# moskewcz/boda

Measured on AMD Instinct MI355X. Metric: effective TFLOP/s (2*M*N*K / time), whole job, higher is better.
Workload: dtype f32

## Files before the change

### boda_amd/csrc/kernels/sgemm_big_f32.hip

```cpp

#ifndef __HIPCC_RTC__
#include <hip/hip_runtime.h>
#endif

typedef float f32x16 __attribute__((ext_vector_type(16)));
typedef float f32x4 __attribute__((ext_vector_type(4)));
typedef unsigned u32x2 __attribute__((ext_vector_type(2)));
#ifndef GROUP_I
#define GROUP_I 8
#endif
#ifndef BKS
#define BKS 8
#endif
#ifndef PF
#define PF 2
#endif
#ifndef TBI
#define TBI 256
#endif
#ifndef TBJ
#define TBJ 256
#endif
#ifndef WI
#define WI 2
#endif
#ifndef WJ
#define WJ 4
#endif
#ifndef MINW
#define MINW 1
#endif
#ifndef MULPRIO
#define MULPRIO 1
#endif
#ifndef STGPRIO
#define STGPRIO 0
#endif
#ifndef NSTG
#define NSTG 4
#endif

struct gemm_args_t {
  float const *I; float const *J; float *D; float const *bias;
  int Mi, Nj, K;
  int ldI, ldJ, ldD;
  int C, H, W, OH, OW;
  int tiles_i, tiles_j;
  int splitk, kt_per;
  float *ws; long ws_slab;
  unsigned I_bytes, J_bytes;
  unsigned D_bytes;
  int out_ctot, out_coff;
  int const *ktab; int ktab_n;
  long bsI, bsJ, bsD;
};

namespace {
constexpr int kNMW = WI * WJ;
static_assert(kNMW == 8 || kNMW == 4, "eight (or four) multiplying waves");
constexpr int kTI = TBI / (WI * 32), kTJ = TBJ / (WJ * 32);
static_assert(TBI % (WI * 32) == 0 && TBJ % (WJ * 32) == 0 && (kTI == 4 || kTI == 2 || kTI == 1) && (kTJ == 2 || kTJ == 1), "wave tile: 4 | 2 | 1 row blocks x 2 | 1 column blocks");
constexpr int kLDI = TBI + 4, kLDJ = TBJ + 4;
constexpr int kImgI = BKS * kLDI, kImgJ = BKS * kLDJ, kImg2 = kImgI + kImgJ;
constexpr int kNLI = BKS * (TBI / 4) / 256, kNLJ = BKS * (TBJ / 4) / 256;
static_assert((BKS * (TBI / 4)) % 256 == 0 && (BKS * (TBJ / 4)) % 256 == 0, "whole float4 units per staging thread");
constexpr int kKK = BKS / 2;
constexpr int kU = (NSTG == 3) ? 3 * PF : ((PF > NSTG) ? PF : NSTG);
constexpr int kD = NSTG - 1;
static_assert(NSTG == 3 || NSTG == 4, "NSTG: 3 | 4");
constexpr int kOOB = (int)0x80000000;
static_assert(BKS % 4 == 0 && (PF == 2 || PF == 4), "BKS % 4 == 0, PF: 2 | 4");
typedef __amdgpu_buffer_rsrc_t rsrc_t;
__device__ __forceinline__ rsrc_t make_rsrc(float const *p, unsigned bytes) { return __builtin_amdgcn_make_buffer_rsrc((void *)p, 0, (int)bytes, 0x00020000); }
__device__ __forceinline__ f32x4 bload4(rsrc_t r, int voff, int soff) { return __builtin_bit_cast(f32x4, __builtin_amdgcn_raw_buffer_load_b128(r, voff, soff, 0)); }
}

#if (TBI / (WI * 32)) == 4
typedef f32x4 avec_t;
#elif (TBI / (WI * 32)) == 2
typedef float2 avec_t;
#else
typedef float avec_t;
#endif
#if (TBJ / (WJ * 32)) == 2
typedef float2 bvec_t;
#else
typedef float bvec_t;
#endif
namespace {
__device__ __forceinline__ float vget(f32x4 const &v, int i) { return v[i]; }
__device__ __forceinline__ float vget(float2 const &v, int i) { return i ? v.y : v.x; }
__device__ __forceinline__ float vget(float const &v, int) { return v; }
}

extern "C" __global__ __launch_bounds__((kNMW + 4) * 64, MINW) void KNAME(gemm_args_t const p) {
  __shared__ __attribute__((aligned(16))) float sm[NSTG * kImg2];
  int const lane = threadIdx.x & 63;
  int const wave = __builtin_amdgcn_readfirstlane(threadIdx.x >> 6);
  bool const stager = wave >= kNMW;

  int tile_i, tile_j;
  {
    int const bid = blockIdx.x, nb = p.tiles_i * p.tiles_j;
    int const q = nb >> 3, rr = nb & 7, xcd = bid & 7, idx = bid >> 3;
    int const nid = ((xcd < rr) ? xcd * (q + 1) : rr * (q + 1) + (xcd - rr) * q) + idx;
    int const group_sz = GROUP_I * p.tiles_j, gid = nid / group_sz, first_i = gid * GROUP_I;
    int const gsz = min(p.tiles_i - first_i, GROUP_I), in_g = nid - gid * group_sz;
    tile_i = first_i + in_g % gsz; tile_j = in_g / gsz;
  }
  int const i0 = tile_i * TBI, j0 = tile_j * TBJ;
  int const nkt = (p.K + BKS - 1) / BKS;
  int const nkt_pad = (nkt + kU - 1) / kU * kU;

  if (stager) {
#if STGPRIO
    __builtin_amdgcn_s_setprio(STGPRIO);
#endif
    int const tid = threadIdx.x - kNMW * 64;
    rsrc_t const rI = make_rsrc(p.I, p.I_bytes), rJ = make_rsrc(p.J, p.J_bytes);
    int goffI[kNLI], goffJ[kNLJ], loffI[kNLI], loffJ[kNLJ], krowI[kNLI], krowJ[kNLJ];
#pragma unroll
    for (int n = 0; n < kNLI; ++n) {
      int const c = tid + n * 256, kr = c / (TBI / 4), x = 4 * (c % (TBI / 4));
      krowI[n] = kr; loffI[n] = kr * kLDI + x;
      goffI[n] = (i0 + x < p.Mi) ? ((kr * p.ldI + i0 + x) * 4) : kOOB;
    }
#pragma unroll
    for (int n = 0; n < kNLJ; ++n) {
      int const c = tid + n * 256, kr = c / (TBJ / 4), x = 4 * (c % (TBJ / 4));
      krowJ[n] = kr; loffJ[n] = kImgI + kr * kLDJ + x;
      goffJ[n] = (j0 + x < p.Nj) ? ((kr * p.ldJ + j0 + x) * 4) : kOOB;
    }
    auto gloadI = [&](int n, int kt) -> f32x4 { return bload4(rI, (kt * BKS + krowI[n] < p.K) ? goffI[n] : kOOB, min(kt, nkt - 1) * (BKS * 4) * p.ldI); };
    auto gloadJ = [&](int n, int kt) -> f32x4 { return bload4(rJ, (kt * BKS + krowJ[n] < p.K) ? goffJ[n] : kOOB, min(kt, nkt - 1) * (BKS * 4) * p.ldJ); };
    auto lstoreI = [&](int n, int stage, f32x4 const &v) { *reinterpret_cast<f32x4 *>(sm + stage * kImg2 + loffI[n]) = v; };
    auto lstoreJ = [&](int n, int stage, f32x4 const &v) { *reinterpret_cast<f32x4 *>(sm + stage * kImg2 + loffJ[n]) = v; };
    f32x4 ringI[PF][kNLI], ringJ[PF][kNLJ];
#pragma unroll
    for (int u = 0; u < PF; ++u) {
#pragma unroll
      for (int n = 0; n < kNLI; ++n) ringI[u][n] = gloadI(n, u);
#pragma unroll
      for (int n = 0; n < kNLJ; ++n) ringJ[u][n] = gloadJ(n, u);
    }
#pragma unroll
    for (int t = 0; t < kD; ++t) {
#pragma unroll
      for (int n = 0; n < kNLI; ++n) { lstoreI(n, t, ringI[t % PF][n]); ringI[t % PF][n] = gloadI(n, t + PF); }
#pragma unroll
      for (int n = 0; n < kNLJ; ++n) { lstoreJ(n, t, ringJ[t % PF][n]); ringJ[t % PF][n] = gloadJ(n, t + PF); }
    }
    asm volatile("s_waitcnt lgkmcnt(0)\n s_barrier" ::: "memory");
    for (int kb = 0; kb < nkt_pad; kb += kU) {
#pragma unroll
      for (int u = 0; u < kU; ++u) {
#pragma unroll
        for (int n = 0; n < kNLI; ++n) { lstoreI(n, (u + kD) % NSTG, ringI[(u + kD) % PF][n]); ringI[(u + kD) % PF][n] = gloadI(n, kb + u + kD + PF); }
#pragma unroll
        for (int n = 0; n < kNLJ; ++n) { lstoreJ(n, (u + kD) % NSTG, ringJ[(u + kD) % PF][n]); ringJ[(u + kD) % PF][n] = gloadJ(n, kb + u + kD + PF); }
        asm volatile("s_waitcnt lgkmcnt(%0)\n s_barrier" :: "n"(kNLI + kNLJ) : "memory");
      }
    }
    return;
  }

#if MULPRIO
  __builtin_amdgcn_s_setprio(MULPRIO);
#endif
  int const wi = wave / WJ, wj = wave % WJ;
  float const *const a_base = sm + (lane >> 5) * kLDI + wi * (kTI * 32) + kTI * (lane & 31);
  float const *const b_base = sm + kImgI + (lane >> 5) * kLDJ + wj * (kTJ * 32) + kTJ * (lane & 31);
  f32x16 acc[kTI][kTJ];
#pragma unroll
  for (int t = 0; t < kTI; ++t)
#pragma unroll
    for (int u = 0; u < kTJ; ++u)
#pragma unroll
      for (int r = 0; r < 16; ++r) acc[t][u][r] = 0.f;

  asm volatile("s_barrier" ::: "memory");
  avec_t a[2]; bvec_t b[2];
  a[0] = *reinterpret_cast<avec_t const *>(a_base); b[0] = *reinterpret_cast<bvec_t const *>(b_base);
  static_assert(kKK % 2 == 0, "an even number of k pairs per step (the operand double buffer carries over from step to step)");
  for (int kb = 0; kb < nkt_pad; kb += kU) {
#pragma unroll
    for (int s = 0; s < kU; ++s) {
      float const *const A = a_base + (s % NSTG) * kImg2, *const B = b_base + (s % NSTG) * kImg2;
      float const *const An = a_base + ((s + 1) % NSTG) * kImg2, *const Bn = b_base + ((s + 1) % NSTG) * kImg2;
#pragma unroll
      for (int kk = 0; kk < kKK; ++kk) {
        if (kk + 1 < kKK) { a[(kk + 1) & 1] = *reinterpret_cast<avec_t const *>(A + (kk + 1) * 2 * kLDI); b[(kk + 1) & 1] = *reinterpret_cast<bvec_t const *>(B + (kk + 1) * 2 * kLDJ); }
#if NSTG == 4
        else { a[0] = *reinterpret_cast<avec_t const *>(An); b[0] = *reinterpret_cast<bvec_t const *>(Bn); }
#endif
        __builtin_amdgcn_sched_barrier(0);
        avec_t const ca = a[kk & 1]; bvec_t const cb = b[kk & 1];
#pragma unroll
        for (int t = 0; t < kTI; ++t)
#pragma unroll
          for (int u = 0; u < kTJ; ++u) acc[t][u] = __builtin_amdgcn_mfma_f32_32x32x2f32(vget(ca, t), vget(cb, u), acc[t][u], 0, 0, 0);
        __builtin_amdgcn_sched_barrier(0);
      }
#if NSTG == 4
      asm volatile("s_barrier" ::: "memory");
#else
      asm volatile("s_waitcnt lgkmcnt(0)\n s_barrier" ::: "memory");
      a[0] = *reinterpret_cast<avec_t const *>(An); b[0] = *reinterpret_cast<bvec_t const *>(Bn);
#endif
    }
  }

  {
    rsrc_t const rD = make_rsrc(p.D, p.D_bytes);
    int const j = j0 + wj * (kTJ * 32) + kTJ * (lane & 31);
    int const il = i0 + wi * (kTI * 32) + kTI * 4 * (lane >> 5);
#pragma unroll
    for (int t = 0; t < kTI; ++t)
#pragma unroll
      for (int r = 0; r < 16; ++r) {
        int const i = il + kTI * ((r & 3) + 8 * (r >> 2)) + t;
        int const off = ((i < p.Mi) && (j < p.Nj)) ? ((i * p.ldD + j) * 4) : kOOB;
#if (TBJ / (WJ * 32)) == 2
        float2 const v = float2{acc[t][0][r], acc[t][1][r]};
        __builtin_amdgcn_raw_buffer_store_b64(__builtin_bit_cast(u32x2, v), rD, off, 0, 0);
#else
        float const v = acc[t][0][r];
        __builtin_amdgcn_raw_buffer_store_b32(__builtin_bit_cast(unsigned, v), rD, off, 0, 0);
#endif
      }
  }
}
```

### boda_amd/csrc/native_internal.h

```cpp
#pragma once
#include "native_kernels.h"
#include <algorithm>
#include <cstdlib>
#include <sstream>

namespace bodahip {

struct gemm_args_t {
  float const *I; float const *J; float *D; float const *bias;
  int Mi, Nj, K;
  int ldI, ldJ, ldD;
  int C, H, W, OH, OW;
  int tiles_i, tiles_j;
  int splitk, kt_per;
  float *ws; long ws_slab;
  unsigned I_bytes, J_bytes;
  unsigned D_bytes;
  int out_ctot, out_coff;
  void const *ktab; int ktab_n;
  long bsI, bsJ, bsD;
};
struct chain_args_t : gemm_args_t {
  float const *I2; float const *bias2; float *Dmid;
  int M2; unsigned I2_bytes, Dmid_bytes;
};
static_assert(sizeof(gemm_args_t) == 176, "gemm_args_t is declared with this size by every kernel source (and by set_kernel_source's text)");

struct kernel_t { hipModule_t mod = nullptr; hipFunction_t func = nullptr; int occ = 0; };

struct native_kernels_t::impl_t {
  std::map<string, kernel_t> kernels;
  std::map<string, string> tune;
  void *ws = nullptr; size_t ws_bytes = 0;
  std::vector<void *> ws_retired;
  std::map<string, void *> ktabs;
  int call_ws_hold = 0;
  size_t call_ws_bytes = 0;
  size_t ts_off = 0, ts_bytes = 0; string ts_hdr;
  hipModule_t wino_mod = nullptr; hipFunction_t wino_filt = nullptr, wino_in = nullptr, wino_out = nullptr, wino_fused = nullptr, wino_filt_t = nullptr;
};


struct plan_t { tile_cfg_t cfg; vect_string defs; string kname; long split_pels = 0; tile_cfg_t tail_cfg; vect_string tail_defs;    bool ipconv = false, k1 = false, bf16 = false, patch = false, stream = false, quad = false, fc = false, big = false, cbig = false, rdec = false, patch16 = false, nhwc = false, nhwc_patch = false, nhwc_multi = false, nhwc_rows = false, ksl = false, bconv_in = false, bconv_filts = false; int rows = 0, cg = 0; };

struct bconv_args_t {
  float const *a; float const *b; float *d;
  float *ws; long ws_slab;
  int B, C, H, W, OC, OH, OW;
  int tiles_i, tiles_j, ksl, kt_per;
  unsigned a_bytes, b_bytes, d_bytes;
};
// ... 50 lines not shown
```

### boda_amd/csrc/native_kernels.cc

```cpp
#include "native_internal.h"

namespace bodahip {

#include "kernels_embed.inc"

native_kernels_t::native_kernels_t(native_host_t *host_) : impl(new impl_t), host(host_) {
  if (char const *e = getenv("BODAHIP_SGEMM_TILE")) impl->tune["sgemm_tile"] = e;
  if (char const *e = getenv("BODAHIP_CONV_TILE")) impl->tune["conv_tile"] = e;
  if (char const *e = getenv("BODAHIP_K1_STREAM")) impl->tune["k1_stream"] = e;
  if (char const *e = getenv("BODAHIP_CONV_ALGO")) impl->tune["conv_algo"] = e;
  if (char const *e = getenv("BODAHIP_EXACT")) impl->tune["exact"] = e;
}
native_kernels_t::~native_kernels_t() {
  if (impl->ts_bytes && impl->ws) {
    char const *e = getenv("BODAHIP_CBIG_TSTAMP"); string fn = e ? string(e) : string(); if (fn.size() > 5 && fn.substr(fn.size() - 5) == ":late") fn.resize(fn.size() - 5);
    std::vector<unsigned long long> h(impl->ts_bytes / 8);
    if (!fn.empty() && hipDeviceSynchronize() == hipSuccess && hipMemcpy(h.data(), (char *)impl->ws + impl->ts_off, impl->ts_bytes, hipMemcpyDeviceToHost) == hipSuccess) {
      if (FILE *f = fopen(fn.c_str(), "a")) { fprintf(f, "%s\n", impl->ts_hdr.c_str());
        for (size_t w = 0; w < h.size() / 16; ++w) { for (int e2 = 0; e2 < 16; ++e2) fprintf(f, "%llu ", h[w * 16 + e2]); fprintf(f, "\n"); } fclose(f); }
    }
  }
  for (auto &kv : impl->kernels) { if (kv.second.mod) (void)hipModuleUnload(kv.second.mod); }
  if (impl->wino_mod) (void)hipModuleUnload(impl->wino_mod);
  if (impl->ws) (void)hipFree(impl->ws);
// ... 10 lines not shown
void native_kernels_t::check_compile_time(rtc_func_info_t const &fi) {
  string const &fn = fi.op.get_func_name();
  if (fn == "hip_sgemm" || fn == "cublas_sgemm" || fn == "hip_sgemm_bf16") return;
  if (fn == "hip_conv" || fn == "cudnn_conv" || fn == "hip_conv_bf16" || fn == "hip_conv_winograd" || fn == "hip_conv_nhwc" || fn == "hip_conv_nhwc_grp" || fn == "hip_conv_nhwc_multi" || fn == "hip_conv_nhwc_set") { (void)fi.op.get_u32("conv_has_relu"); return; }
  if (fn == "hip_conv_k1_chain") { (void)fi.op.get_u32("conv_has_relu"); (void)fi.op.get_u32("conv_has_relu2"); return; }
  if (fn == "hip_conv_filts_kmajor") return;
  if (fn == "hip_bconv_in" || fn == "hip_bconv_filts" || fn == "hip_bconv_biases") {
    for (char const *an : {"in", "filts", "out_grad_loss", "stride", "in_pad"}) (void)fi.op.get_dims(an);
    return;
  }
  rt_err("unknown/unhandled native hip function: " + fn);
}
void native_kernels_t::set_tune(string const &key, string const &val) {
  if (key != "sgemm_tile" && key != "conv_tile" && key != "k1_stream" && key != "conv_algo" && key != "exact") rt_err("set_tune: unknown key '" + key + "'");
  if (key == "exact" && !val.empty() && val != "0" && val != "1") rt_err("set_tune: exact must be 0 | 1");
  if (key == "conv_algo" && !val.empty() && val != "direct" && val != "winograd" && val != "winograd_all") rt_err("set_tune: conv_algo must be direct | winograd | winograd_all");
  if (val.empty()) impl->tune.erase(key); else { impl->tune[key] = val; }
}


void launch(native_host_t *host, kernel_t &k, gemm_args_t &a, tile_cfg_t const &c) {
  void *params[] = {&a};
  uint32_t const grid = (uint32_t)a.tiles_i * (uint32_t)a.tiles_j * (uint32_t)std::max(1, a.splitk);
  hip_err_chk(host->nh_launch(k.func, grid, 1, (uint32_t)c.threads(), params), "hipModuleLaunchKernel(native)");
}


std::vector<char> compile_plan(plan_t const &p, string const &arch, string *log) {
  vect_string opts = p.defs; opts.push_back("-DKNAME=" + p.kname);
  return hiprtc_compile(p.bconv_in ? k_src_bconv_in_f32 : p.bconv_filts ? k_src_bconv_filts_f32 : p.nhwc_rows ? k_src_conv_nhwc_rows_bf16 : p.nhwc_multi ? k_src_conv_nhwc_multi_bf16 : p.nhwc_patch ? k_src_conv_nhwc_patch_bf16 : p.nhwc ? k_src_conv_nhwc_bf16 : p.patch16 ? k_src_conv_patch_bf16 : (p.cbig ? k_src_conv_big_f32 : p.big ? k_src_sgemm_big_f32 : p.fc ? k_src_fc_f32 : p.stream ? (p.quad ? k_src_k1_quad_f32 : k_src_k1_stream_f32) : (p.bf16 ? k_src_gemm_conv_bf16 : k_src_gemm_conv_f32)), p.kname, arch, opts, log, true);
}

void ensure_ws(native_kernels_t::impl_t *impl, native_host_t *host, size_t need) {
  if (impl->ws_bytes >= need) return;
  if (host->nh_capturing()) rt_err("graph capture: kernel workspace not allocated yet -- run the call list once before capturing it");
  if (impl->ws) {
    hip_err_chk(hipStreamSynchronize(host->nh_stream()), "hipStreamSynchronize");
    if (host->nh_live_graphs() > 0) impl->ws_retired.push_back(impl->ws); else hip_err_chk(hipFree(impl->ws), "hipFree");
    impl->ws = nullptr; impl->ws_bytes = 0;
  }
  hip_err_chk(hipMalloc(&impl->ws, need), "hipMalloc(kernel scratch)"); impl->ws_bytes = need;
}
static void setup_splitk(native_kernels_t::impl_t *impl, native_host_t *host, gemm_args_t &ga, tile_cfg_t const &cfg, size_t out_elems) {
  ga.splitk = cfg.SPLITK; ga.kt_per = 0; ga.ws = nullptr; ga.ws_slab = 0;
  if (cfg.SPLITK <= 1) { ga.splitk = 1; return; }
  int const nkt = (ga.K + cfg.BK - 1) / cfg.BK;
  ga.kt_per = (nkt + cfg.SPLITK - 1) / cfg.SPLITK;
// ... 113 lines not shown
  void *d = nullptr;
  hip_err_chk(hipMalloc(&d, h.size() * sizeof(int)), "hipMalloc(rtab)");
  hip_err_chk(hipMemcpyAsync(d, h.data(), h.size() * sizeof(int), hipMemcpyHostToDevice, host->nh_stream()), "hipMemcpyAsync(rtab)");
  hip_err_chk(hipStreamSynchronize(host->nh_stream()), "hipStreamSynchronize");
  impl->ktabs.emplace(key, d);
  return ktab_t{d, (int)n};
}

string tune_of(native_kernels_t::impl_t *impl, char const *key) { auto t = impl->tune.find(key); return (t == impl->tune.end()) ? string() : t->second; }

static void sgemm_parts(native_kernels_t *nk, native_kernels_t::impl_t *impl, native_host_t *host, float const *a, float const *b, float *c, uint32_t M, uint32_t N, uint32_t K, std::vector<sgemm_part_t> const &parts) {
  if ((uint64_t)K * M * 4 > 0x80000000ull || (uint64_t)K * N * 4 > 0x80000000ull || (uint64_t)M * N * 4 >= 0x7ffffff0ull) unsup_err("hip_sgemm: operands / c of 2 GiB or more are not supported (32-bit buffer offsets)");
  uint32_t grid = 0; bool first = true;
  for (sgemm_part_t const &q : parts) {
    plan_t const p = plan_sgemm(q.rows, q.cols, K, host->nh_num_cus(), q.tile, false);
    kernel_t &k = get_kernel(impl, host, p);
    gemm_args_t ga; memset(&ga, 0, sizeof(ga));
    ga.I = a + q.m0; ga.J = b + q.n0; ga.D = c + (size_t)q.m0 * N + q.n0; ga.bias = nullptr;
    ga.Mi = (int)q.rows; ga.Nj = (int)q.cols; ga.K = (int)K; ga.ldI = (int)M; ga.ldJ = (int)N; ga.ldD = (int)N;
    ga.I_bytes = (unsigned)(((uint64_t)K * M - q.m0) * 4); ga.J_bytes = (unsigned)(((uint64_t)K * N - q.n0) * 4); ga.D_bytes = (unsigned)((((uint64_t)q.rows - 1) * N + q.cols) * 4);
    ga.tiles_i = (int)((q.rows + p.cfg.BI - 1) / p.cfg.BI); ga.tiles_j = (int)((q.cols + p.cfg.BJ - 1) / p.cfg.BJ); ga.splitk = 1;
    launch(host, k, ga, p.cfg);
    grid += (uint32_t)ga.tiles_i * ga.tiles_j;
    if (first) { nk->last_launch.kernel = p.kname; nk->last_launch.cfg = p.cfg; nk->last_launch.block = p.cfg.threads(); first = false; }
  }
  nk->last_launch.grid = grid; nk->last_launch.flops = 2.0 * M * N * K; nk->last_launch.algo_bytes = 4.0 * ((double)K * M + (double)K * N + (double)M * N);
}

void native_kernels_t::sgemm(float const *a, float const *b, float *c, uint32_t M, uint32_t N, uint32_t K, bool bf16, bool half) {
  if (!M || !N) return;
  size_t const esz = half ? 2 : 4;
  if (half && bf16) unsup_err("hip_sgemm_bf16: half-typed tensors are not supported (bf16 OPERANDS are made from float tensors)");
  if (!K) { hip_err_chk(hipMemsetAsync(c, 0, (size_t)M * N * esz, host->nh_stream()), "hipMemsetAsync"); return; }
  if (M > 0x7fffffffu || N > 0x7fffffffu || K > 0x7fffffffu) unsup_err("hip_sgemm: dims exceed int32");
  string tile_for;
  if (char const *e = getenv("BODAHIP_SGEMM_TILE_FOR")) {
    string const key = std::to_string(M) + "="; string const v = e; size_t const at = (";" + v).find(";" + key);
    if (M == N && N == K && at != string::npos) { size_t const b = at + key.size(), en = v.find(';', b); tile_for = v.substr(b, en == string::npos ? string::npos : en - b); }
  }
  if (!bf16 && !half && tune_of(impl, "sgemm_tile").empty() && tile_for.empty() && M % 4 == 0 && N % 4 == 0) {
    std::vector<sgemm_part_t> parts;
    if (!parse_parts_env(M, N, K, parts)) parts = plan_sgemm_parts(M, N, K, host->nh_num_cus());
    if (!parts.empty()) { sgemm_parts(this, impl, host, a, b, c, M, N, K, parts); return; }
  }
  if (!bf16 && !half && tune_of(impl, "sgemm_tile").empty() && tile_for.empty()) tile_for = sgemm_wide_tile(M, N, K, host->nh_num_cus());
  if (!bf16 && !half && tune_of(impl, "sgemm_tile").empty() && tile_for.empty()) {
    sgemm_split_t const sp = plan_sgemm_split(M, N, K, host->nh_num_cus());
    if (sp.m_main) {
      if ((uint64_t)K * M * 4 > 0x80000000ull || (uint64_t)K * N * 4 > 0x80000000ull || (uint64_t)M * N * 4 >= 0x7ffffff0ull) unsup_err("hip_sgemm: operands / c of 2 GiB or more are not supported (32-bit buffer offsets)");
      uint32_t grid = 0;
      for (int part = 0; part < 2; ++part) {
        uint32_t const m0 = part ? sp.m_main : 0, rows = part ? M - sp.m_main : sp.m_main;
        plan_t const p = plan_sgemm(rows, N, K, host->nh_num_cus(), part ? sp.tail_tile : string(kBigTile), false);
        kernel_t &k = get_kernel(impl, host, p);
        gemm_args_t ga; memset(&ga, 0, sizeof(ga));
        ga.I = a + m0; ga.J = b; ga.D = c + (size_t)m0 * N; ga.bias = nullptr;
        ga.Mi = (int)rows; ga.Nj = (int)N; ga.K = (int)K; ga.ldI = (int)M; ga.ldJ = (int)N; ga.ldD = (int)N;
        ga.I_bytes = (unsigned)(((uint64_t)K * M - m0) * 4); ga.J_bytes = (unsigned)((uint64_t)K * N * 4); ga.D_bytes = (unsigned)((uint64_t)rows * N * 4);
        ga.tiles_i = (int)((rows + p.cfg.BI - 1) / p.cfg.BI); ga.tiles_j = (int)((N + p.cfg.BJ - 1) / p.cfg.BJ); ga.splitk = 1;
        launch(host, k, ga, p.cfg);
        grid += (uint32_t)ga.tiles_i * ga.tiles_j;
        if (!part) { last_launch.kernel = p.kname; last_launch.cfg = p.cfg; last_launch.block = p.cfg.threads(); }
      }
      last_launch.grid = grid; last_launch.flops = 2.0 * M * N * K; last_launch.algo_bytes = 4.0 * ((double)K * M + (double)K * N + (double)M * N);
      return;
    }
  }
  plan_t p = plan_sgemm(M, N, K, host->nh_num_cus(), tile_for.empty() ? tune_of(impl, "sgemm_tile") : tile_for, bf16, 1, !half);
  if (half) {
    if (p.cfg.SPLITK > 1) unsup_err("hip_sgemm: split-K tiles are not supported for half-typed tensors");
    p.kname = "bodahip_sgemm_f16s"; p.defs.push_back("-DHALF=1");
  }
  tile_cfg_t const &cfg = p.cfg;
  kernel_t &k = get_kernel(impl, host, p);
  gemm_args_t ga; memset(&ga, 0, sizeof(ga));
  ga.I = a; ga.J = b; ga.D = c; ga.bias = nullptr;
  ga.Mi = (int)M; ga.Nj = (int)N; ga.K = (int)K; ga.ldI = (int)M; ga.ldJ = (int)N; ga.ldD = (int)N;
  if ((uint64_t)K * M * 4 > 0x80000000ull || (uint64_t)K * N * 4 > 0x80000000ull) unsup_err("hip_sgemm: operands larger than 2 GiB are not supported (32-bit buffer offsets)");
  ga.I_bytes = (unsigned)((uint64_t)K * M * esz); ga.J_bytes = (unsigned)((uint64_t)K * N * esz);
  if ((uint64_t)M * N * 4 >= 0x7ffffff0ull) unsup_err("hip_sgemm: c of 2 GiB or more is not supported (32-bit store offsets, masked lanes use offset 2^31)");
  ga.D_bytes = (unsigned)((uint64_t)M * N * esz);
  ga.tiles_i = (int)((M + cfg.BI - 1) / cfg.BI); ga.tiles_j = (int)((N + cfg.BJ - 1) / cfg.BJ);
  setup_splitk(impl, host, ga, cfg, (size_t)M * N);
  launch(host, k, ga, cfg);
  if (cfg.SPLITK > 1) reduce_splitk(impl, host, ga, (long)M * N, false, false, 1, 1);
  last_launch.kernel = p.kname; last_launch.cfg = cfg; last_launch.grid = (uint32_t)ga.tiles_i * ga.tiles_j * cfg.SPLITK; last_launch.block = cfg.threads();
  last_launch.flops = 2.0 * M * N * K; last_launch.algo_bytes = (double)esz * ((double)K * M + (double)K * N + (double)M * N);
}

static void launch_patch16(native_kernels_t::impl_t *impl, native_host_t *host, plan_t const &p, kernel_t &k, gemm_args_t &ga, float const *filts,
                           conv_geom_t const &g, size_t ws_off) {
  int const taps = g.KH * g.KW, ncg = (g.C + 7) / 8;
  size_t const fbytes = (size_t)ncg * taps * g.OC * 16;
  if (fbytes >= 0x7ffffff0ull) unsup_err("hip_conv_bf16: re-laid-out filters of 2 GiB or more");
  if (impl->ws_bytes < ws_off + fbytes) ensure_ws(impl, host, ws_off + fbytes);
  plan_t fp; fp.patch16 = true; fp.bf16 = true; fp.kname = "bodahip_filt_bf16"; fp.defs = {"-DFILT_ONLY=1"};
  kernel_t &fk = get_kernel(impl, host, fp);
  gemm_args_t fa; memset(&fa, 0, sizeof(fa));
  fa.I = filts; fa.D = (float *)((char *)impl->ws + ws_off); fa.Mi = g.OC; fa.C = g.C; fa.K = taps;
  void *fparams[] = {&fa};
  long const nchunks = (long)ncg * taps * g.OC;
  hip_err_chk(host->nh_launch(fk.func, (uint32_t)((nchunks + 255) / 256), 1, 256, fparams), "hipModuleLaunchKernel(filt_bf16)");
  ga.I = (float const *)((char *)impl->ws + ws_off); ga.I_bytes = (unsigned)fbytes;
  void *params[] = {&ga};
  hip_err_chk(host->nh_launch(k.func, (uint32_t)(ga.tiles_i * ga.tiles_j), 1, (uint32_t)p.cfg.threads(), params), "hipModuleLaunchKernel(conv_patch_bf16)");
}

struct s2d_args_t { float const *src; float *dst; int B, C, H, W, OC, KH, KW; int S, C2, H2, W2; int oy, ox; int filt; int mode, c2_lo; };
bool s2d_geom(conv_geom_t const &g, conv_geom_t &g2, int &pry, int &prx) {
// ... 306 lines not shown
  ga.tiles_i = 1; ga.tiles_j = (int)(((long)g.B * ((g.OH * g.OW + 127) / 128) + cfg.WJ - 1) / cfg.WJ);
  long const slots = std::max(1l, (long)host->nh_num_cus());
  long const per = (ga.tiles_j + slots - 1) / slots;
  ga.kt_per = (int)((ga.tiles_j + per - 1) / per); ga.splitk = 1;
  if (ga.kt_per >= 8) ga.kt_per = (ga.kt_per + 7) / 8 * 8;
  void *params[] = {&ga};
  hip_err_chk(host->nh_launch(k.func, (uint32_t)ga.kt_per, 1, (uint32_t)cfg.threads(), params), "hipModuleLaunchKernel(k1_chain)");
  last_launch.kernel = p.kname; last_launch.cfg = cfg; last_launch.grid = (uint32_t)ga.kt_per; last_launch.block = cfg.threads();
  last_launch.flops = 2.0 * Nj * ((double)g.OC * g.C + (double)oc2 * g.OC);
  last_launch.algo_bytes = 4.0 * ((double)g.B * g.C * g.H * g.W + (double)Nj * oc2 + (double)g.OC * g.C + g.OC + (double)oc2 * g.OC + oc2);
}


kernel_t &get_kernel(native_kernels_t::impl_t *impl, native_host_t *host, plan_t const &p) {
  string key = p.kname; for (auto const &d : p.defs) key += " " + d;
  auto it = impl->kernels.find(key);
  if (it != impl->kernels.end()) return it->second;
  if (host->nh_capturing()) rt_err("graph capture: native kernel '" + key + "' is not specialised yet -- run the call list once before capturing it");
  string log;
  std::vector<char> code = compile_plan(p, host->nh_arch(), &log);
  kernel_t k;
  hip_err_chk(hipModuleLoadData(&k.mod, code.data()), "hipModuleLoadData(native)");
  hip_err_chk(hipModuleGetFunction(&k.func, k.mod, p.kname.c_str()), "hipModuleGetFunction(native)");
  return impl->kernels.emplace(key, k).first->second;
}



static bconv_args_t bconv_args(conv_geom_t const &g) {
  bconv_args_t a; memset(&a, 0, sizeof(a));
  a.B = g.B; a.C = g.C; a.H = g.H; a.W = g.W; a.OC = g.OC; a.OH = g.OH; a.OW = g.OW;
  return a;
}
void native_kernels_t::bconv_in(float const *filts, float const *out_grad, float *in_grad, conv_geom_t const &g) {
  plan_t const p = plan_bconv_in(g, host->nh_num_cus(), tune_of(impl, "conv_tile"));
  kernel_t &k = get_kernel(impl, host, p);
  bconv_args_t a = bconv_args(g);
  a.a = filts; a.b = out_grad; a.d = in_grad;
  a.a_bytes = (unsigned)(4ull * g.OC * g.C * g.KH * g.KW); a.b_bytes = (unsigned)(4ull * g.B * g.OC * g.OH * g.OW); a.d_bytes = (unsigned)(4ull * g.B * g.C * g.H * g.W);
  a.tiles_i = (g.C + p.cfg.BI - 1) / p.cfg.BI; a.tiles_j = (int)bconv_in_tiles(g, p.cfg.BJ); a.ksl = 1;
  uint32_t const grid = (uint32_t)a.tiles_i * (uint32_t)a.tiles_j;
  void *params[] = {&a};
  if (grid) hip_err_chk(host->nh_launch(k.func, grid, 1, (uint32_t)p.cfg.threads(), params), "hipModuleLaunchKernel(bconv_in)");
  int const TY = (g.KH + g.SY - 1) / g.SY, TX = (g.KW + g.SX - 1) / g.SX;
  last_launch.kernel = p.kname; last_launch.cfg = p.cfg; last_launch.grid = grid; last_launch.block = p.cfg.threads();
  last_launch.flops = 2.0 * g.B * g.H * g.W * g.C * ((double)g.OC * TY * TX);
// ... 49 lines not shown
```

### boda_amd/csrc/native_plan.cc

```cpp
#include "native_internal.h"

namespace bodahip {

bool parse_tile(string const &s, tile_cfg_t &c) {
  int v[11] = {0, 0, 0, 0, 0, 0, 0, 0, 0, 0, 0}; int n = 0; string cur;
  for (size_t i = 0; i <= s.size(); ++i) {
    if (i == s.size() || s[i] == 'x' || s[i] == ':') { if (cur.empty() || n >= 11) return false; v[n++] = atoi(cur.c_str()); cur.clear(); }
    else if (s[i] >= '0' && s[i] <= '9') cur.push_back(s[i]); else return false;
  }
  if (n < 5) return false;
  c.BI = v[0]; c.BJ = v[1]; c.BK = v[2]; c.WI = v[3]; c.WJ = v[4]; c.MINW = (n >= 6) ? v[5] : 1; c.SPLITK = (n >= 7) ? v[6] : 1; c.MT = (n >= 8) ? v[7] : 32; c.PF = (n >= 9) ? v[8] : 1; c.SW = (n >= 10) ? v[9] : 0; c.KHO = (n >= 11) ? v[10] : 0;
  return true;
}
static void check_cfg(tile_cfg_t const &c, bool gather, bool patch = false) {
  int const nt = c.WI * c.WJ * 64;
  bool ok = c.BI > 0 && c.BJ > 0 && c.BK > 0 && c.WI > 0 && c.WJ > 0 && nt <= 1024 && c.threads() <= 1024 && (c.MT == 32 || c.MT == 16) && (c.BI % (c.WI * c.MT) == 0) && (c.BJ % (c.WJ * c.MT) == 0) &&
            (c.BK % 2 == 0) && (c.MT == 32 || c.BK % 4 == 0) && (c.BI % 4 == 0) && (c.BJ % 4 == 0);
  if (gather) ok = ok && ((c.BK * c.BJ) % nt == 0);
  if (gather) ok = ok && (nt % c.BJ == 0) && (c.BJ % 64 == 0);
  ok = ok && c.SPLITK >= 1 && c.SPLITK <= 64 && c.MINW >= 1 && (c.PF == 1 || c.PF == 2 || c.PF == 4 || c.PF == 6 || c.PF == 8);
  ok = ok && c.KHO >= 0 && c.KHO <= 64 && (c.KHO <= 1 || (c.SPLITK == 1 && c.SW == 0));
  if (c.PF > 2) ok = ok && ((long)c.PF * c.BK * (c.BI + c.BJ) / nt <= 192);
  int const accs = (c.BI / (c.WI * c.MT)) * (c.BJ / (c.WJ * c.MT));
  ok = ok && accs * (c.MT == 32 ? 16 : 4) <= 256;
// ... 113 lines not shown
  if (c.MT != 32) { c.MT = 32; c.BI = 64; c.BJ = 64; c.WI = 2; c.WJ = 2; }
  if (c.BK != 32 && c.BK != 64) c.BK = 32;
  c.PF = 1;
  if (!explicit_tile) {
    c.SPLITK = 1;
    if (Mi > 0 && num_cus > 0 && getenv("BODAHIP_NO_BF16_SPLITK") == nullptr) {
      long const nkt = (K + c.BK - 1) / c.BK;
      long const tiles = ((Mi + c.BI - 1) / c.BI) * ((Nj + c.BJ - 1) / c.BJ), tiles128 = ((Mi + 127) / 128) * ((Nj + 127) / 128);
      if (tiles <= num_cus && nkt >= 64) {
        long s = std::min<long>(16, (2l * num_cus + tiles128 - 1) / tiles128);
        s = std::min<long>(s, nkt / 8);
        if (s >= 2) { c.BI = 128; c.BJ = 128; c.WI = 2; c.WJ = 2; c.MINW = 2; c.SPLITK = (int)s; }
      }
    }
  }
  int const nt = c.threads();
  bool ok = (c.BI % (c.WI * 32) == 0) && (c.BJ % (c.WJ * 32) == 0) && ((c.BI * c.BK / 8) % nt == 0) && ((c.BJ * c.BK / 8) % nt == 0) && nt <= 1024 &&
            (c.BI / (c.WI * 32)) * (c.BJ / (c.WJ * 32)) * 16 <= 256 && 4ull * (c.BK + 8) * (c.BI + c.BJ) <= 160 * 1024;
  if (gather) ok = ok && (c.BJ % 64 == 0) && (nt % c.BJ == 0);
  if (!ok) unsup_err("native bf16 kernel: unsupported tile configuration " + c.str());
}

static char const *const kStg64 = "64x64x16x2x2x4x1x32x2x3";
plan_t plan_sgemm(uint32_t M, uint32_t N, uint32_t K, int num_cus, string const &tile, bool bf16, int batch, bool allow_big) {
  plan_t p; p.kname = bf16 ? "bodahip_sgemm_bf16" : "bodahip_sgemm_f32"; p.bf16 = bf16;
  p.cfg = choose_cfg((int)M, (int)std::min<uint64_t>((uint64_t)N * batch, 0x7fffffffull), (int)K, num_cus, false, bf16);
  if (!tile.empty()) { if (!parse_tile(tile, p.cfg)) rt_err("bad sgemm_tile '" + tile + "'"); }
  if (bf16) {
    bf16_cfg(p.cfg, false, M, N, K, num_cus, !tile.empty());
    p.defs = cfg_defs(p.cfg); p.defs.push_back("-DI_MODE=0"); p.defs.push_back("-DJ_MODE=0"); p.defs.push_back("-DEPI=0");
    if (p.cfg.SPLITK > 1) p.defs.push_back("-DSPLITK=1");
    return p;
  }
  if (!tile.empty() && p.cfg.SW == 3) {
    tile_cfg_t const &c = p.cfg;
    int const nmw = c.WI * c.WJ, ti = (c.WI > 0 && c.BI % (c.WI * 32) == 0) ? c.BI / (c.WI * 32) : 0, tj = (c.WJ > 0 && c.BJ % (c.WJ * 32) == 0) ? c.BJ / (c.WJ * 32) : 0;
    bool const ok = (nmw == 8 || nmw == 4) && (ti == 4 || ti == 2 || ti == 1) && (tj == 2 || tj == 1) && c.BK >= 4 && c.BK <= 32 && c.BK % 4 == 0 && (c.BK * (c.BI / 4)) % 256 == 0 &&
                    (c.BK * (c.BJ / 4)) % 256 == 0 && (c.PF == 2 || c.PF == 4) && c.MT == 32 && c.SPLITK == 1 && c.MINW >= 1 && c.MINW <= 8 && 4l * 4 * c.BK * (c.BI + c.BJ + 8) <= 160 * 1024;
    if (!ok || batch != 1 || M % 4 || N % 4 || !allow_big) unsup_err("hip_sgemm: unsupported staging-wave tile " + c.str() + " (8 | 4 multiplying waves of 4 | 2 | 1 x 2 | 1 blocks, whole float4 units per staging thread, M and N multiples of 4)");
    p.big = true; p.kname = "bodahip_sgemm_big_f32"; p.cfg.KHO = 0;
    p.defs = {"-DBKS=" + std::to_string(c.BK), "-DPF=" + std::to_string(c.PF), "-DTBI=" + std::to_string(c.BI), "-DTBJ=" + std::to_string(c.BJ), "-DWI=" + std::to_string(c.WI),
              "-DWJ=" + std::to_string(c.WJ), "-DMINW=" + std::to_string(c.MINW)};
    if (char const *x = getenv("BODAHIP_EXTRA_DEFS")) { std::istringstream is(x); string tok; while (is >> tok) p.defs.push_back(tok); }
    return p;
  }
  bool const big_tile = (p.cfg.BI == 256 || p.cfg.BI == 128) && (p.cfg.BJ == 256 || p.cfg.BJ == 128);
  bool const want_big = big_tile && ((p.cfg.WI == 3 && p.cfg.WJ == 4) || (p.cfg.BI == 256 && p.cfg.BJ == 256));
  if (allow_big && batch == 1 && want_big && p.cfg.MT == 32 && p.cfg.SPLITK == 1 && M % 4 == 0 && N % 4 == 0) {
    char const *e = getenv("BODAHIP_SGEMM_BIG");
    if (!(e && string(e) == "off")) {
      int bks = 8, pf = 4;
      if (!tile.empty() && p.cfg.WI == 3 && p.cfg.BK >= 4 && p.cfg.BK <= 32 && p.cfg.BK % 4 == 0) bks = p.cfg.BK;
      if (e && *e) { if (sscanf(e, "%dx%d", &bks, &pf) != 2 || bks < 4 || bks > 32 || bks % 4 || (pf != 2 && pf != 4)) rt_err(string("bad BODAHIP_SGEMM_BIG '") + e + "' (off | BKSxPF)"); }
      if (bks * (p.cfg.BI / 4) % 256 || bks * (p.cfg.BJ / 4) % 256) bks = 8;
      int const minw = (p.cfg.BI == 128 && p.cfg.BJ == 128) ? ((!tile.empty() && p.cfg.MINW >= 1) ? std::min(p.cfg.MINW, 2) : 2) : 1;
      p.big = true; p.kname = "bodahip_sgemm_big_f32"; p.cfg.BK = bks; p.cfg.PF = pf; p.cfg.WI = 3; p.cfg.WJ = 4; p.cfg.MINW = minw;
      p.defs = {"-DBKS=" + std::to_string(bks), "-DPF=" + std::to_string(pf)};
      if (!(p.cfg.BI == 256 && p.cfg.BJ == 256)) {
        bool const tall = (p.cfg.BI == 256 && p.cfg.BJ == 128);
        p.defs.push_back("-DTBI=" + std::to_string(p.cfg.BI)); p.defs.push_back("-DTBJ=" + std::to_string(p.cfg.BJ));
        p.defs.push_back(string("-DWI=") + (tall ? "4" : "2")); p.defs.push_back(string("-DWJ=") + (tall ? "2" : "4")); p.defs.push_back("-DMINW=" + std::to_string(minw));
      }
      if (char const *x = getenv("BODAHIP_EXTRA_DEFS")) { std::istringstream is(x); string tok; while (is >> tok) p.defs.push_back(tok); }
      return p;
    }
  }
  if (tile.empty() && allow_big && batch == 1 && p.cfg.BI == 64 && p.cfg.BJ == 64 && p.cfg.MT == 32 && p.cfg.SPLITK == 1 && M % 4 == 0 && N % 4 == 0 && K >= 512 && getenv("BODAHIP_NO_SGEMM_STG64") == nullptr) {
    char const *e = getenv("BODAHIP_SGEMM_BIG");
    if (!(e && string(e) == "off")) return plan_sgemm(M, N, K, num_cus, kStg64, false, 1, true);
  }
  p.cfg.KHO = 0;
  check_cfg(p.cfg, false);
  p.defs = cfg_defs(p.cfg);
  p.defs.push_back(string("-DI_MODE=") + ((M % 4 == 0) ? "0" : "1"));
  p.defs.push_back(string("-DJ_MODE=") + ((N % 4 == 0) ? "0" : "1"));
  p.defs.push_back("-DEPI=0");
  if (p.cfg.SPLITK > 1) p.defs.push_back("-DSPLITK=1");
  return p;
}
bool plan_patch_bf16(conv_geom_t const &g, int num_cus, plan_t &p) {
  if (getenv("BODAHIP_NO_PATCH16")) return false;
  int const taps = g.KH * g.KW;
  if (!(g.SX == 1 && taps >= 2 && g.KH >= g.SY && g.C % 8 == 0 && g.C >= 16)) return false;
  if (g.OH == 1 && g.OW == 1 && g.PY == 0 && g.PX == 0 && g.KH == g.H && g.KW == g.W) return false;
  int cg = 1; while (cg * taps < 16) ++cg;
// ... 761 lines not shown
```

Measured before the change: 144.6.

## Stage SGEMM tiles with buffer-load-to-LDS DMA from the compute waves

```diff
diff --git a/boda_amd/csrc/kernels/sgemm_big_f32.hip b/boda_amd/csrc/kernels/sgemm_big_f32.hip
--- a/boda_amd/csrc/kernels/sgemm_big_f32.hip
+++ b/boda_amd/csrc/kernels/sgemm_big_f32.hip
@@ -35,6 +35,24 @@
 #endif
 #ifndef STGPRIO
 #define STGPRIO 0
+#endif
+#ifndef LDSDMA
+#define LDSDMA 0
+#endif
+#ifndef ABLATE
+#define ABLATE 0
+#endif
+#ifndef TSTAMP
+#define TSTAMP 0
+#endif
+#if LDSDMA && defined(DMA_NSTG)
+#define NSTG DMA_NSTG
+#endif
+#ifndef DMASPLIT
+#define DMASPLIT 0
+#endif
+#ifndef DMAPRIO
+#define DMAPRIO 0
 #endif
 #ifndef NSTG
 #define NSTG 4
@@ -60,19 +78,31 @@
 static_assert(kNMW == 8 || kNMW == 4, "eight (or four) multiplying waves");
 constexpr int kTI = TBI / (WI * 32), kTJ = TBJ / (WJ * 32);
 static_assert(TBI % (WI * 32) == 0 && TBJ % (WJ * 32) == 0 && (kTI == 4 || kTI == 2 || kTI == 1) && (kTJ == 2 || kTJ == 1), "wave tile: 4 | 2 | 1 row blocks x 2 | 1 column blocks");
-constexpr int kLDI = TBI + 4, kLDJ = TBJ + 4;
+constexpr int kPad = LDSDMA ? 0 : 4;
+constexpr int kLDI = TBI + kPad, kLDJ = TBJ + kPad;
 constexpr int kImgI = BKS * kLDI, kImgJ = BKS * kLDJ, kImg2 = kImgI + kImgJ;
 constexpr int kNLI = BKS * (TBI / 4) / 256, kNLJ = BKS * (TBJ / 4) / 256;
 static_assert((BKS * (TBI / 4)) % 256 == 0 && (BKS * (TBJ / 4)) % 256 == 0, "whole float4 units per staging thread");
 constexpr int kKK = BKS / 2;
-constexpr int kU = (NSTG == 3) ? 3 * PF : ((PF > NSTG) ? PF : NSTG);
+constexpr int kU = LDSDMA ? NSTG : (NSTG == 3) ? 3 * PF : ((PF > NSTG) ? PF : NSTG);
 constexpr int kD = NSTG - 1;
-static_assert(NSTG == 3 || NSTG == 4, "NSTG: 3 | 4");
+static_assert(NSTG == 3 || NSTG == 4 || (LDSDMA && NSTG >= 3 && NSTG <= 6), "NSTG: 3 | 4 (LDS-DMA: 3 .. 6)");
+constexpr int kNSW = LDSDMA ? 0 : 4;
+constexpr int kShI = BKS * TBI * 4 / kNMW, kShJ = BKS * TBJ * 4 / kNMW;
+constexpr int kLnI = kShI >= 1024 ? 64 : kShI / 16, kLnJ = kShJ >= 1024 ? 64 : kShJ / 16;
+constexpr int kNI = kShI / (kLnI * 16), kNJ = kShJ / (kLnJ * 16);
+constexpr int kL = kNI + kNJ;
+static_assert(!LDSDMA || (kNMW == 8 && TBI == 256 && (TBJ == 256 || TBJ == 128) && (kShI % 1024 == 0 || kShI == 512) && (kShJ % 1024 == 0 || kShJ == 512)), "LDS-DMA: the 256 x 256 and 256 x 128 forms, whole 512-byte shares per wave");
+static_assert(!LDSDMA || (kD - 1) * kL <= 63, "loads kept in flight must fit the 6-bit vmcnt");
+typedef __attribute__((address_space(3))) void *lds_t;
 constexpr int kOOB = (int)0x80000000;
 static_assert(BKS % 4 == 0 && (PF == 2 || PF == 4), "BKS % 4 == 0, PF: 2 | 4");
 typedef __amdgpu_buffer_rsrc_t rsrc_t;
 __device__ __forceinline__ rsrc_t make_rsrc(float const *p, unsigned bytes) { return __builtin_amdgcn_make_buffer_rsrc((void *)p, 0, (int)bytes, 0x00020000); }
 __device__ __forceinline__ f32x4 bload4(rsrc_t r, int voff, int soff) { return __builtin_bit_cast(f32x4, __builtin_amdgcn_raw_buffer_load_b128(r, voff, soff, 0)); }
+__device__ __forceinline__ void dma16(rsrc_t r, unsigned lds, int voff, int soff) {
+  asm volatile("s_nop 0\n\tbuffer_load_dwordx4 %0, %2, %3 offen lds" :: "v"(voff), "{m0}"(lds), "s"(r), "s"(soff) : "memory");
+}
 }
 
 #if (TBI / (WI * 32)) == 4
@@ -93,11 +123,20 @@
 __device__ __forceinline__ float vget(float const &v, int) { return v; }
 }
 
-extern "C" __global__ __launch_bounds__((kNMW + 4) * 64, MINW) void KNAME(gemm_args_t const p) {
+#if LDSDMA
+#define BODAHIP_SGEMM_MINWAVES (TBJ == 128 ? 4 : 2)
+#else
+#define BODAHIP_SGEMM_MINWAVES MINW
+#endif
+extern "C" __global__ __launch_bounds__((kNMW + kNSW) * 64, BODAHIP_SGEMM_MINWAVES) void KNAME(gemm_args_t const p) {
   __shared__ __attribute__((aligned(16))) float sm[NSTG * kImg2];
   int const lane = threadIdx.x & 63;
   int const wave = __builtin_amdgcn_readfirstlane(threadIdx.x >> 6);
-  bool const stager = wave >= kNMW;
+  bool const stager = !LDSDMA && wave >= kNMW;
+  if (LDSDMA && wave >= kNMW) return;
+#if TSTAMP
+  unsigned long long const ts_rt0 = __builtin_amdgcn_s_memrealtime(), ts_mt0 = __builtin_amdgcn_s_memtime();
+#endif
 
   int tile_i, tile_j;
   {
@@ -131,10 +170,21 @@
       krowJ[n] = kr; loffJ[n] = kImgI + kr * kLDJ + x;
       goffJ[n] = (j0 + x < p.Nj) ? ((kr * p.ldJ + j0 + x) * 4) : kOOB;
     }
+#if ABLATE & 2
+    auto gen = [&](int n, int kt) -> f32x4 { float const v = (float)((tid + n * 7 + kt * 13) & 15) * 0.25f - 2.f; return f32x4{v, v + 1.f, v - 1.f, 0.5f * v}; };
+    auto gloadI = [&](int n, int kt) -> f32x4 { return gen(n, kt); };
+    auto gloadJ = [&](int n, int kt) -> f32x4 { return gen(n + 5, kt); };
+#else
     auto gloadI = [&](int n, int kt) -> f32x4 { return bload4(rI, (kt * BKS + krowI[n] < p.K) ? goffI[n] : kOOB, min(kt, nkt - 1) * (BKS * 4) * p.ldI); };
     auto gloadJ = [&](int n, int kt) -> f32x4 { return bload4(rJ, (kt * BKS + krowJ[n] < p.K) ? goffJ[n] : kOOB, min(kt, nkt - 1) * (BKS * 4) * p.ldJ); };
+#endif
+#if ABLATE & 4
+    auto lstoreI = [&](int, int, f32x4 const &v) { asm volatile("" :: "v"(v)); };
+    auto lstoreJ = [&](int, int, f32x4 const &v) { asm volatile("" :: "v"(v)); };
+#else
     auto lstoreI = [&](int n, int stage, f32x4 const &v) { *reinterpret_cast<f32x4 *>(sm + stage * kImg2 + loffI[n]) = v; };
     auto lstoreJ = [&](int n, int stage, f32x4 const &v) { *reinterpret_cast<f32x4 *>(sm + stage * kImg2 + loffJ[n]) = v; };
+#endif
     f32x4 ringI[PF][kNLI], ringJ[PF][kNLJ];
 #pragma unroll
     for (int u = 0; u < PF; ++u) {
@@ -178,7 +228,47 @@
 #pragma unroll
       for (int r = 0; r < 16; ++r) acc[t][u][r] = 0.f;
 
+#if LDSDMA
+  constexpr int kEarly = NSTG >= 4 ? 1 : 0;
+  constexpr int kWait = (kD - 1 - kEarly) * kL;
+  static_assert(kD - 1 - kEarly >= 1, "a counted vmcnt, never 0 inside the K loop");
+  rsrc_t const rI = make_rsrc(p.I, p.I_bytes), rJ = make_rsrc(p.J, p.J_bytes);
+  int goffI[kNI], krI[kNI], goffJ[kNJ], krJ[kNJ];
+#pragma unroll
+  for (int n = 0; n < kNI; ++n) {
+    int const f = (wave * kShI + n * kLnI * 16) / 4 + lane * 4, kr = f / TBI, x = f % TBI;
+    krI[n] = kr; goffI[n] = (i0 + x < p.Mi) ? ((kr * p.ldI + i0 + x) * 4) : kOOB;
+  }
+#pragma unroll
+  for (int n = 0; n < kNJ; ++n) {
+    int const f = (wave * kShJ + n * kLnJ * 16) / 4 + lane * 4, kr = f / TBJ, x = f % TBJ;
+    krJ[n] = kr; goffJ[n] = (j0 + x < p.Nj) ? ((kr * p.ldJ + j0 + x) * 4) : kOOB;
+  }
+  unsigned const lds0 = __builtin_amdgcn_readfirstlane((unsigned)(unsigned long)(lds_t)sm);
+  auto dma = [&](int kt, int stage, int part) {
+#if !(ABLATE & 2)
+#if DMAPRIO
+    __builtin_amdgcn_s_setprio(DMAPRIO);
+#endif
+    int const sI = min(kt, nkt - 1) * (BKS * 4) * p.ldI, sJ = min(kt, nkt - 1) * (BKS * 4) * p.ldJ;
+#pragma unroll
+    for (int n = 0; n < kNI; ++n)
+      if ((part & 1) && (kLnI == 64 || lane < kLnI)) dma16(rI, lds0 + (stage * kImg2) * 4 + wave * kShI + n * kLnI * 16, (kt * BKS + krI[n] < p.K) ? goffI[n] : kOOB, sI);
+#pragma unroll
+    for (int n = 0; n < kNJ; ++n)
+      if ((part & 2) && (kLnJ == 64 || lane < kLnJ)) dma16(rJ, lds0 + (stage * kImg2 + kImgI) * 4 + wave * kShJ + n * kLnJ * 16, (kt * BKS + krJ[n] < p.K) ? goffJ[n] : kOOB, sJ);
+#if DMAPRIO
+    __builtin_amdgcn_s_setprio(MULPRIO);
+#endif
+#endif
+  };
+#pragma unroll
+  for (int t = 0; t < kD; ++t) dma(t, t, 3);
+  asm volatile("s_waitcnt vmcnt(%0)\n s_barrier" :: "n"(kWait) : "memory");
+#else
   asm volatile("s_barrier" ::: "memory");
+  constexpr int kEarly = NSTG == 4 ? 1 : 0;
+#endif
   avec_t a[2]; bvec_t b[2];
   a[0] = *reinterpret_cast<avec_t const *>(a_base); b[0] = *reinterpret_cast<bvec_t const *>(b_base);
   static_assert(kKK % 2 == 0, "an even number of k pairs per step (the operand double buffer carries over from step to step)");
@@ -189,10 +279,12 @@
       float const *const An = a_base + ((s + 1) % NSTG) * kImg2, *const Bn = b_base + ((s + 1) % NSTG) * kImg2;
 #pragma unroll
       for (int kk = 0; kk < kKK; ++kk) {
+#if LDSDMA
+        if (kk == 0) dma(kb + s + kD, (s + kD) % NSTG, DMASPLIT ? 1 : 3);
+        if (DMASPLIT && kk == kKK / 2) dma(kb + s + kD, (s + kD) % NSTG, 2);
+#endif
         if (kk + 1 < kKK) { a[(kk + 1) & 1] = *reinterpret_cast<avec_t const *>(A + (kk + 1) * 2 * kLDI); b[(kk + 1) & 1] = *reinterpret_cast<bvec_t const *>(B + (kk + 1) * 2 * kLDJ); }
-#if NSTG == 4
-        else { a[0] = *reinterpret_cast<avec_t const *>(An); b[0] = *reinterpret_cast<bvec_t const *>(Bn); }
-#endif
+        else if (kEarly) { a[0] = *reinterpret_cast<avec_t const *>(An); b[0] = *reinterpret_cast<bvec_t const *>(Bn); }
         __builtin_amdgcn_sched_barrier(0);
         avec_t const ca = a[kk & 1]; bvec_t const cb = b[kk & 1];
 #pragma unroll
@@ -201,14 +293,24 @@
           for (int u = 0; u < kTJ; ++u) acc[t][u] = __builtin_amdgcn_mfma_f32_32x32x2f32(vget(ca, t), vget(cb, u), acc[t][u], 0, 0, 0);
         __builtin_amdgcn_sched_barrier(0);
       }
-#if NSTG == 4
-      asm volatile("s_barrier" ::: "memory");
-#else
-      asm volatile("s_waitcnt lgkmcnt(0)\n s_barrier" ::: "memory");
-      a[0] = *reinterpret_cast<avec_t const *>(An); b[0] = *reinterpret_cast<bvec_t const *>(Bn);
-#endif
-    }
-  }
+#if LDSDMA
+      asm volatile("s_waitcnt vmcnt(%0) lgkmcnt(0)\n s_barrier" :: "n"(kWait) : "memory");
+#else
+      if (kEarly) asm volatile("s_barrier" ::: "memory");
+      else asm volatile("s_waitcnt lgkmcnt(0)\n s_barrier" ::: "memory");
+#endif
+      if (!kEarly) { a[0] = *reinterpret_cast<avec_t const *>(An); b[0] = *reinterpret_cast<bvec_t const *>(Bn); }
+    }
+  }
+#if LDSDMA
+  asm volatile("s_waitcnt vmcnt(0)" ::: "memory");
+#endif
+#if TSTAMP
+  if (threadIdx.x == 0 && p.ws) {
+    unsigned long long *const ts = reinterpret_cast<unsigned long long *>(p.ws) + (long)blockIdx.x * 16;
+    ts[1] = __builtin_amdgcn_s_memrealtime(); ts[3] = __builtin_amdgcn_s_memtime(); ts[0] = ts_rt0; ts[2] = ts_mt0; ts[4] = __builtin_amdgcn_s_getreg((20 << 0) | (0 << 6) | (3 << 11));
+  }
+#endif
 
   {
     rsrc_t const rD = make_rsrc(p.D, p.D_bytes);
@@ -220,6 +322,7 @@
       for (int r = 0; r < 16; ++r) {
         int const i = il + kTI * ((r & 3) + 8 * (r >> 2)) + t;
         int const off = ((i < p.Mi) && (j < p.Nj)) ? ((i * p.ldD + j) * 4) : kOOB;
+        if (ABLATE & 1) { asm volatile("" :: "v"(acc[t][0][r]), "v"(acc[t][kTJ - 1][r])); continue; }
 #if (TBJ / (WJ * 32)) == 2
         float2 const v = float2{acc[t][0][r], acc[t][1][r]};
         __builtin_amdgcn_raw_buffer_store_b64(__builtin_bit_cast(u32x2, v), rD, off, 0, 0);
diff --git a/boda_amd/csrc/native_internal.h b/boda_amd/csrc/native_internal.h
--- a/boda_amd/csrc/native_internal.h
+++ b/boda_amd/csrc/native_internal.h
@@ -26,7 +26,8 @@
 };
 static_assert(sizeof(gemm_args_t) == 176, "gemm_args_t is declared with this size by every kernel source (and by set_kernel_source's text)");
 
-struct kernel_t { hipModule_t mod = nullptr; hipFunction_t func = nullptr; int occ = 0; };
+struct kernel_t { hipModule_t mod = nullptr; hipFunction_t func = nullptr; int occ = 0; int threads = 0; };
+inline int block_of(kernel_t const &k, tile_cfg_t const &c) { return k.threads ? k.threads : c.threads(); }
 
 struct native_kernels_t::impl_t {
   std::map<string, kernel_t> kernels;
diff --git a/boda_amd/csrc/native_kernels.cc b/boda_amd/csrc/native_kernels.cc
--- a/boda_amd/csrc/native_kernels.cc
+++ b/boda_amd/csrc/native_kernels.cc
@@ -56,7 +56,7 @@
 void launch(native_host_t *host, kernel_t &k, gemm_args_t &a, tile_cfg_t const &c) {
   void *params[] = {&a};
   uint32_t const grid = (uint32_t)a.tiles_i * (uint32_t)a.tiles_j * (uint32_t)std::max(1, a.splitk);
-  hip_err_chk(host->nh_launch(k.func, grid, 1, (uint32_t)c.threads(), params), "hipModuleLaunchKernel(native)");
+  hip_err_chk(host->nh_launch(k.func, grid, 1, (uint32_t)block_of(k, c), params), "hipModuleLaunchKernel(native)");
 }
 
 
@@ -216,7 +216,7 @@
     ga.tiles_i = (int)((q.rows + p.cfg.BI - 1) / p.cfg.BI); ga.tiles_j = (int)((q.cols + p.cfg.BJ - 1) / p.cfg.BJ); ga.splitk = 1;
     launch(host, k, ga, p.cfg);
     grid += (uint32_t)ga.tiles_i * ga.tiles_j;
-    if (first) { nk->last_launch.kernel = p.kname; nk->last_launch.cfg = p.cfg; nk->last_launch.block = p.cfg.threads(); first = false; }
+    if (first) { nk->last_launch.kernel = p.kname; nk->last_launch.cfg = p.cfg; nk->last_launch.block = block_of(k, p.cfg); first = false; }
   }
   nk->last_launch.grid = grid; nk->last_launch.flops = 2.0 * M * N * K; nk->last_launch.algo_bytes = 4.0 * ((double)K * M + (double)K * N + (double)M * N);
 }
@@ -254,7 +254,7 @@
         ga.tiles_i = (int)((rows + p.cfg.BI - 1) / p.cfg.BI); ga.tiles_j = (int)((N + p.cfg.BJ - 1) / p.cfg.BJ); ga.splitk = 1;
         launch(host, k, ga, p.cfg);
         grid += (uint32_t)ga.tiles_i * ga.tiles_j;
-        if (!part) { last_launch.kernel = p.kname; last_launch.cfg = p.cfg; last_launch.block = p.cfg.threads(); }
+        if (!part) { last_launch.kernel = p.kname; last_launch.cfg = p.cfg; last_launch.block = block_of(k, p.cfg); }
       }
       last_launch.grid = grid; last_launch.flops = 2.0 * M * N * K; last_launch.algo_bytes = 4.0 * ((double)K * M + (double)K * N + (double)M * N);
       return;
@@ -278,7 +278,7 @@
   setup_splitk(impl, host, ga, cfg, (size_t)M * N);
   launch(host, k, ga, cfg);
   if (cfg.SPLITK > 1) reduce_splitk(impl, host, ga, (long)M * N, false, false, 1, 1);
-  last_launch.kernel = p.kname; last_launch.cfg = cfg; last_launch.grid = (uint32_t)ga.tiles_i * ga.tiles_j * cfg.SPLITK; last_launch.block = cfg.threads();
+  last_launch.kernel = p.kname; last_launch.cfg = cfg; last_launch.grid = (uint32_t)ga.tiles_i * ga.tiles_j * cfg.SPLITK; last_launch.block = block_of(k, cfg);
   last_launch.flops = 2.0 * M * N * K; last_launch.algo_bytes = (double)esz * ((double)K * M + (double)K * N + (double)M * N);
 }
 
@@ -631,6 +631,7 @@
   kernel_t k;
   hip_err_chk(hipModuleLoadData(&k.mod, code.data()), "hipModuleLoadData(native)");
   hip_err_chk(hipModuleGetFunction(&k.func, k.mod, p.kname.c_str()), "hipModuleGetFunction(native)");
+  if (p.big && std::find(p.defs.begin(), p.defs.end(), "-DLDSDMA=1") != p.defs.end()) k.threads = 8 * 64;
   return impl->kernels.emplace(key, k).first->second;
 }
 
diff --git a/boda_amd/csrc/native_plan.cc b/boda_amd/csrc/native_plan.cc
--- a/boda_amd/csrc/native_plan.cc
+++ b/boda_amd/csrc/native_plan.cc
@@ -159,6 +159,13 @@
 }
 
 static char const *const kStg64 = "64x64x16x2x2x4x1x32x2x3";
+static char const *const kSgemmDmaDefault = "on";
+static bool sgemm_dma(int tbj) {
+  char const *e = getenv("BODAHIP_SGEMM_DMA"); string const v = (e && *e) ? e : kSgemmDmaDefault;
+  if (v != "off" && v != "on" && v != "256x256") rt_err("bad BODAHIP_SGEMM_DMA '" + v + "' (off | on | 256x256)");
+  return v == "on" || (v == "256x256" && tbj == 256);
+}
+
 plan_t plan_sgemm(uint32_t M, uint32_t N, uint32_t K, int num_cus, string const &tile, bool bf16, int batch, bool allow_big) {
   plan_t p; p.kname = bf16 ? "bodahip_sgemm_bf16" : "bodahip_sgemm_f32"; p.bf16 = bf16;
   p.cfg = choose_cfg((int)M, (int)std::min<uint64_t>((uint64_t)N * batch, 0x7fffffffull), (int)K, num_cus, false, bf16);
@@ -198,6 +205,7 @@
         p.defs.push_back("-DTBI=" + std::to_string(p.cfg.BI)); p.defs.push_back("-DTBJ=" + std::to_string(p.cfg.BJ));
         p.defs.push_back(string("-DWI=") + (tall ? "4" : "2")); p.defs.push_back(string("-DWJ=") + (tall ? "2" : "4")); p.defs.push_back("-DMINW=" + std::to_string(minw));
       }
+      if (p.cfg.BI == 256 && bks % 8 == 0 && sgemm_dma(p.cfg.BJ)) p.defs.push_back("-DLDSDMA=1");
       if (char const *x = getenv("BODAHIP_EXTRA_DEFS")) { std::istringstream is(x); string tok; while (is >> tok) p.defs.push_back(tok); }
       return p;
     }
```

Result: faster. 146.5 (median of 6 runs) (+1.3%).
